# RuntimeRacer/vall-e

Hardware: AMD Instinct MI355X
Metric: AR codec-tokens/sec/GPU + NAR 7-stage p50 latency, d=1024 L=12 10s utterance (higher is better)
Workload: dtype bf16

## Files before the change

vall-e_amd/csrc/common.hpp:

```cpp
#pragma once
#include <hip/hip_runtime.h>
#include <stdint.h>

#ifdef VX_STAMPS
extern __device__ unsigned long long g_vx_stamps[32];
#define VX_STAMP(i)                                                                                        \
  do {                                                                                                     \
    if (blockIdx.x == 0 && blockIdx.y == 0 && blockIdx.z == 0 && threadIdx.x == 0) g_vx_stamps[i] = wall_clock64(); \
  } while (0)
extern __device__ unsigned long long* g_vx_kstamps;
#define VX_KSTAMP_WG(kid, st_ptr)                                                                                  \
  do {                                                                                                             \
    if ((kid) >= 0 && (kid) < 64 && blockIdx.x == gridDim.x - 1) {                                                 \
      unsigned long long* vx_r_ = g_vx_kstamps;                                                                    \
      if (vx_r_ != nullptr && threadIdx.x == 0)                                                                    \
        vx_r_[(size_t)(((st_ptr)->pass) & 15) * 64 + (kid)] = __builtin_amdgcn_s_memrealtime();                   \
      return;                                                                                                      \
    }                                                                                                              \
  } while (0)
#define VX_KSTAMP_SELF(kid, pass, t0)                                                                              \
  do {                                                                                                             \
    unsigned long long* vx_r_ = g_vx_kstamps;                                                                      \
    if (vx_r_ != nullptr && (kid) >= 0 && (kid) < 64 && threadIdx.x == 0) vx_r_[(size_t)((pass) & 15) * 64 + (kid)] = (t0); \
  } while (0)
constexpr int VX_KSTAMP_EXTRA = 1;
#else
#define VX_STAMP(i) do { } while (0)
#define VX_KSTAMP_WG(kid, st_ptr) do { } while (0)
#define VX_KSTAMP_SELF(kid, pass, t0) do { } while (0)
constexpr int VX_KSTAMP_EXTRA = 0;
#endif

namespace vx {

inline int vx_cur_device() {
  int d = 0;
  (void)hipGetDevice(&d);
  return (d < 0 || d >= 16) ? 0 : d;
}
inline int vx_cu_count() {
  static int cu[16] = {};
  const int d = vx_cur_device();
  if (cu[d] <= 0) {
    int n = 256;
    (void)hipDeviceGetAttribute(&n, hipDeviceAttributeMultiprocessorCount, d);
    cu[d] = n > 0 ? n : 256;
  }
  return cu[d];
// ... 10 lines not shown
__device__ __forceinline__ float to_f32(bf16 v) { return (float)v; }
template <typename T> __device__ __forceinline__ T from_f32(float v);
template <> __device__ __forceinline__ float from_f32<float>(float v) { return v; }
template <> __device__ __forceinline__ bf16 from_f32<bf16>(float v) { return (bf16)v; }

template <typename T> struct Vec16;
template <> struct Vec16<float> { static constexpr int N = 4; };
template <> struct Vec16<bf16> { static constexpr int N = 8; };

__device__ __forceinline__ void unpack16(const uint4& r, float (&o)[4], float*) {
  o[0] = __uint_as_float(r.x); o[1] = __uint_as_float(r.y); o[2] = __uint_as_float(r.z); o[3] = __uint_as_float(r.w);
}
__device__ __forceinline__ void unpack16(const uint4& r, float (&o)[8], bf16*) {
  o[0] = __uint_as_float(r.x << 16); o[1] = __uint_as_float(r.x & 0xffff0000u);
  o[2] = __uint_as_float(r.y << 16); o[3] = __uint_as_float(r.y & 0xffff0000u);
  o[4] = __uint_as_float(r.z << 16); o[5] = __uint_as_float(r.z & 0xffff0000u);
  o[6] = __uint_as_float(r.w << 16); o[7] = __uint_as_float(r.w & 0xffff0000u);
}
template <typename T> __device__ __forceinline__ void unpack(const uint4& r, float (&o)[Vec16<T>::N]) {
  unpack16(r, o, (T*)nullptr);
}
template <typename T> __device__ __forceinline__ uint4 ld16(const T* p) { return *reinterpret_cast<const uint4*>(p); }
typedef unsigned vx_u32x4 __attribute__((ext_vector_type(4)));

template <int CTRL, int ROW_MASK = 0xF> __device__ __forceinline__ float dpp_f(float old, float v) {
  return __builtin_bit_cast(float, __builtin_amdgcn_update_dpp(__builtin_bit_cast(int, old), __builtin_bit_cast(int, v),
                                                                CTRL, ROW_MASK, 0xF, false));
}
template <int CTRL, int ROW_MASK = 0xF> __device__ __forceinline__ int dpp_i(int old, int v) {
  return __builtin_amdgcn_update_dpp(old, v, CTRL, ROW_MASK, 0xF, false);
}
__device__ __forceinline__ float lane63(float v) {
  return __builtin_bit_cast(float, __builtin_amdgcn_readlane(__builtin_bit_cast(int, v), 63));
}
__device__ __forceinline__ float wave_sum_dpp(float v) {
  v += dpp_f<0xB1>(0.f, v);
  v += dpp_f<0x4E>(0.f, v);
  v += dpp_f<0x124>(0.f, v);
  v += dpp_f<0x128>(0.f, v);
  v += dpp_f<0x142, 0xA>(0.f, v);
  v += dpp_f<0x143, 0xC>(0.f, v);
  return lane63(v);
}
__device__ __forceinline__ float wave_max_dpp(float v) {
  v = fmaxf(v, dpp_f<0xB1>(v, v));
  v = fmaxf(v, dpp_f<0x4E>(v, v));
// ... 127 lines not shown
```

vall-e_amd/csrc/engine.hip:

```cpp
#include <hip/hip_runtime.h>

#include <cmath>
#include <cstdarg>
#include <cstdio>
#include <array>
#include <cstring>
#include <string>
#include <type_traits>
#include <unordered_map>
#include <vector>

#include "host.hpp"
#ifdef VX_STAMPS
__device__ unsigned long long g_vx_stamps[32];
__device__ unsigned long long* g_vx_kstamps = nullptr;
__device__ unsigned long long* g_fq_stamps = nullptr;
#endif
#include "ar_kernels.hpp"
#include "ar_tp.hpp"
#include "rows_kernels.hpp"
#include "mfma_kernels.hpp"
#include "batch_kernels.hpp"
#include "mx_kernels.hpp"
#include "logprob.hpp"
#include "align.hpp"

using namespace vx;

static thread_local std::string g_err;
int vx::fail(int code, const char* fmt, ...) {
  char buf[512];
  va_list ap;
  va_start(ap, fmt);
  vsnprintf(buf, sizeof buf, fmt, ap);
  va_end(ap);
  g_err = buf;
  return code;
}

// ... 3296 lines not shown
```

vall-e_amd/csrc/mfma_kernels.hpp:

```cpp
#pragma once
#include <cstdlib>
#include <type_traits>
#include <unordered_map>

#include "common.hpp"
#include "rows_kernels.hpp"

namespace vx {

typedef __bf16 bf16x8_t __attribute__((ext_vector_type(8)));
typedef float f32x16_t __attribute__((ext_vector_type(16)));

template <int EPI, bool OUT_F32, int RING>
__global__ __launch_bounds__(256) void mfma_gemm_kernel(const bf16* __restrict__ A, const bf16* __restrict__ W,
                                                        const float* __restrict__ bias, void* __restrict__ Cv, int M,
                                                        int N, int K, bf16* __restrict__ vt, int vt_n0, int vt_ld, int ld) {
  const int bx = blockIdx.x, by = blockIdx.y, bz = blockIdx.z;
  A += (size_t)bz * K;
  W += (size_t)bz * K;
  if (OUT_F32) Cv = reinterpret_cast<float*>(Cv) + (size_t)bz * M * N;
  constexpr int BM = 128, BN = 128;
  extern __shared__ __attribute__((aligned(16))) unsigned char lds[];
  const int tid = threadIdx.x, lane = tid & 63, wave = tid >> 6;
  const int wm = wave >> 1, wn = wave & 1;
  const int r = lane & 31, h = lane >> 5;
  const int m0 = by * BM, n0 = bx * BN;

  f32x16_t acc[2][2];
#pragma unroll
  for (int i = 0; i < 2; ++i)
#pragma unroll
    for (int j = 0; j < 2; ++j)
#pragma unroll
      for (int v = 0; v < 16; ++v) acc[i][j][v] = 0.f;
  float bias_r[2] = {0.f, 0.f};
  if (EPI != GE_PLAIN) {
#pragma unroll
    for (int j = 0; j < 2; ++j) bias_r[j] = bias[min(n0 + wn * 64 + j * 32 + r, N - 1)];
  }

  constexpr int RK = RING;
  constexpr int RB = RK * 2;
  constexpr int CPR = RB / 16;
  constexpr int KS = RK / 16;
  constexpr int OPB = BM * RB;
  constexpr int NI = OPB / 4096;
  constexpr int ND = 2 * NI;
  auto swz = [](int row) { return RB == 128 ? ((row >> 1) & 7) : ((0 - (row >> 2)) & 3); };
  const int nk = K / RK;
  const int row0 = tid / CPR;
  const int csrc = ((tid % CPR) ^ swz(row0)) * 8;
  const bf16 *sA[NI], *sW[NI];
#pragma unroll
  for (int i = 0; i < NI; ++i) {
    sA[i] = A + (size_t)min(m0 + row0 + (256 / CPR) * i, M - 1) * ld + csrc;
    sW[i] = W + (size_t)min(n0 + row0 + (256 / CPR) * i, N - 1) * ld + csrc;
  }
  const int dbase = (tid - lane) * 16;
  auto stage = [&](int st) {
    unsigned char* base = lds + (st & 3) * (2 * OPB);
    const int k0 = st * RK;
#pragma unroll
    for (int i = 0; i < NI; ++i)
      __builtin_amdgcn_global_load_lds((const __attribute__((address_space(1))) void*)(sA[i] + k0),
                                       (__attribute__((address_space(3))) void*)(base + dbase + 4096 * i), 16, 0, 0);
#pragma unroll
    for (int i = 0; i < NI; ++i)
      __builtin_amdgcn_global_load_lds((const __attribute__((address_space(1))) void*)(sW[i] + k0),
                                       (__attribute__((address_space(3))) void*)(base + OPB + dbase + 4096 * i), 16, 0, 0);
  };
  bf16x8_t fa0[KS][2], fb0[KS][2], fa1[KS][2], fb1[KS][2];
  auto lread = [&](int st, bf16x8_t (&fa)[KS][2], bf16x8_t (&fb)[KS][2]) {
    const unsigned char* ba = lds + (st & 3) * (2 * OPB);
    const unsigned char* bw = ba + OPB;
#pragma unroll
    for (int ks = 0; ks < KS; ++ks)
#pragma unroll
      for (int i = 0; i < 2; ++i) {
        const int row = wm * 64 + i * 32 + r;
        fa[ks][i] = *reinterpret_cast<const bf16x8_t*>(ba + row * RB + (((ks * 2 + h) ^ swz(row)) << 4));
        const int col = wn * 64 + i * 32 + r;
        fb[ks][i] = *reinterpret_cast<const bf16x8_t*>(bw + col * RB + (((ks * 2 + h) ^ swz(col)) << 4));
      }
  };
  auto mm = [&](const bf16x8_t (&fa)[KS][2], const bf16x8_t (&fb)[KS][2]) {
#pragma unroll
    for (int ks = 0; ks < KS; ++ks)
#pragma unroll
      for (int i = 0; i < 2; ++i)
#pragma unroll
        for (int j = 0; j < 2; ++j) acc[i][j] = __builtin_amdgcn_mfma_f32_32x32x16_bf16(fa[ks][i], fb[ks][j], acc[i][j], 0, 0, 0);
  };
  auto steady = [&](int st, bf16x8_t (&fa)[KS][2], bf16x8_t (&fb)[KS][2], bf16x8_t (&na)[KS][2], bf16x8_t (&nb)[KS][2]) {
    stage(st + 3);
    lread(st + 1, na, nb);
    mm(fa, fb);
#pragma unroll
    for (int i = 0; i < ND; ++i) {
      __builtin_amdgcn_sched_group_barrier(0x010, 1, 0);
      __builtin_amdgcn_sched_group_barrier(0x008, 1, 0);
    }
#pragma unroll
    for (int i = 0; i < 4 * KS - ND; ++i) {
      __builtin_amdgcn_sched_group_barrier(0x100, 4 * KS / (4 * KS - ND), 0);
      __builtin_amdgcn_sched_group_barrier(0x008, 1, 0);
    }
    if (ND == 8) asm volatile("s_waitcnt vmcnt(8)\n\ts_barrier" ::: "memory");
    else asm volatile("s_waitcnt vmcnt(4)\n\ts_barrier" ::: "memory");
  };
  auto tail = [&](int st, bf16x8_t (&fa)[KS][2], bf16x8_t (&fb)[KS][2], bf16x8_t (&na)[KS][2], bf16x8_t (&nb)[KS][2]) {
    const bool more = st + 3 < nk;
    if (more) stage(st + 3);
    if (st + 1 < nk) lread(st + 1, na, nb);
    mm(fa, fb);
    if (more && ND == 8) asm volatile("s_waitcnt vmcnt(8)\n\ts_barrier" ::: "memory");
    else if (more) asm volatile("s_waitcnt vmcnt(4)\n\ts_barrier" ::: "memory");
    else asm volatile("s_waitcnt vmcnt(0)\n\ts_barrier" ::: "memory");
  };
  VX_STAMP(0);
  const int pre = nk < 3 ? nk : 3;
  for (int st = 0; st < pre; ++st) stage(st);
  VX_STAMP(1);
  if (pre == 3 && ND == 8) asm volatile("s_waitcnt vmcnt(8)\n\ts_barrier" ::: "memory");
  else if (pre == 3) asm volatile("s_waitcnt vmcnt(4)\n\ts_barrier" ::: "memory");
  else asm volatile("s_waitcnt vmcnt(0)\n\ts_barrier" ::: "memory");
  lread(0, fa0, fb0);
  VX_STAMP(2);
  int st = 0;
  for (; st + 4 < nk; st += 2) {
    steady(st, fa0, fb0, fa1, fb1);
    steady(st + 1, fa1, fb1, fa0, fb0);
  }
  VX_STAMP(3);
  for (; st < nk; st += 2) {
    tail(st, fa0, fb0, fa1, fb1);
    if (st + 1 < nk) tail(st + 1, fa1, fb1, fa0, fb0);
  }
  VX_STAMP(4);
  asm volatile("" : "+v"(bias_r[0]), "+v"(bias_r[1]));

  if constexpr (!OUT_F32) {
    constexpr int LDT = 136;
    bf16* tile = reinterpret_cast<bf16*>(lds);
#pragma unroll
    for (int j = 0; j < 2; ++j) {
      const int nl = wn * 64 + j * 32 + r;
      const float bv = bias_r[j];
#pragma unroll
      for (int i = 0; i < 2; ++i)
#pragma unroll
        for (int v = 0; v < 16; ++v) {
          const int ml = wm * 64 + i * 32 + (v & 3) + 8 * (v >> 2) + 4 * h;
          float x = acc[i][j][v] + bv;
          if (EPI == GE_RELU) x = fmaxf(x, 0.f);
          tile[ml * LDT + nl] = (bf16)x;
        }
    }
    __syncthreads();
    bf16* C = reinterpret_cast<bf16*>(Cv);
#pragma unroll
    for (int q = 0; q < 8; ++q) {
      const int id = tid + 256 * q, row = id >> 4, c = id & 15;
      if (m0 + row < M)
        *reinterpret_cast<uint4*>(C + (size_t)(m0 + row) * N + n0 + c * 8) = *reinterpret_cast<const uint4*>(tile + row * LDT + c * 8);
    }
    if (vt != nullptr && n0 >= vt_n0) {
#pragma unroll
      for (int q = 0; q < 8; ++q) {
        const int id = tid + 256 * q, nl = id >> 4, mc = id & 15;
        union { bf16 e[8]; uint4 u; } pk;
#pragma unroll
        for (int k = 0; k < 8; ++k) pk.e[k] = tile[(mc * 8 + k) * LDT + nl];
        *reinterpret_cast<uint4*>(vt + (size_t)(n0 + nl - vt_n0) * vt_ld + m0 + mc * 8) = pk.u;
      }
    }
  } else if (m0 + BM <= M && n0 + BN <= N) {
    float* cbase = reinterpret_cast<float*>(Cv) + (size_t)(m0 + wm * 64 + 4 * h) * N + n0 + wn * 64 + r;
    float old[2][2][16];
    if (EPI == GE_RESID) {
#pragma unroll
      for (int j = 0; j < 2; ++j)
#pragma unroll
        for (int i = 0; i < 2; ++i)
#pragma unroll
          for (int v = 0; v < 16; ++v) old[i][j][v] = cbase[(size_t)(i * 32 + (v & 3) + 8 * (v >> 2)) * N + j * 32];
    }
#pragma unroll
    for (int j = 0; j < 2; ++j) {
      const float bv = bias_r[j];
#pragma unroll
      for (int i = 0; i < 2; ++i)
#pragma unroll
        for (int v = 0; v < 16; ++v) {
          float x = acc[i][j][v] + bv;
          if (EPI == GE_RELU) x = fmaxf(x, 0.f);
          if (EPI == GE_RESID) x += old[i][j][v];
          cbase[(size_t)(i * 32 + (v & 3) + 8 * (v >> 2)) * N + j * 32] = x;
        }
    }
  } else {
#pragma unroll
    for (int j = 0; j < 2; ++j) {
      const int n = n0 + wn * 64 + j * 32 + r;
      const float bv = bias_r[j];
#pragma unroll
      for (int i = 0; i < 2; ++i) {
#pragma unroll
        for (int v = 0; v < 16; ++v) {
          const int m = m0 + wm * 64 + i * 32 + (v & 3) + 8 * (v >> 2) + 4 * h;
          if (m < M && n < N) {
            float x = acc[i][j][v] + bv;
            if (EPI == GE_RELU) x = fmaxf(x, 0.f);
            float* c = reinterpret_cast<float*>(Cv) + (size_t)m * N + n;
            *c = (EPI == GE_RESID) ? (*c + x) : x;
          }
        }
      }
    }
  }
  VX_STAMP(5);
}

template <int EPI, bool OUT_F32, int SPLITK>
__global__ __launch_bounds__(256) void wgemm_kernel(const bf16* __restrict__ A, const bf16* __restrict__ W,
                                                    const float* __restrict__ bias, void* __restrict__ Cv, int M, int N,
                                                    int K, bf16* __restrict__ vt, int vt_n0, int vt_ld, int ngroups,
                                                    int ngroups_pad) {
  extern __shared__ __attribute__((aligned(16))) unsigned char lds[];
  const int tid = threadIdx.x, lane = tid & 63, wave = tid >> 6;
  const int r = lane & 31, h = lane >> 5;
  const int ng = blockIdx.x % ngroups_pad, mt = blockIdx.x / ngroups_pad;
  if (ng >= ngroups) return;
  const int m0 = mt * 64;
  const int n0 = (SPLITK == 1) ? (ng * 4 + wave) * 64 : ng * 64;
  const int kbeg = (SPLITK == 1) ? 0 : wave * (K / SPLITK);
  const int nk = (K / SPLITK) / 64;
  unsigned char* my = lds + wave * 32768;
  const bool active = n0 < N;

  f32x16_t acc[2][2];
#pragma unroll
  for (int i = 0; i < 2; ++i)
#pragma unroll
// ... 582 lines not shown
    };
    if (is_tail) {
      unsigned lo = (unsigned)((r * 256 + 4 * g) * 4);
      asm volatile("" : "+v"(lo));
      unsigned char* slab = reinterpret_cast<unsigned char*>(tl.ws + (size_t)(tail_a * S + tail_s) * 65536 + wr * 32768 + wc * 64) + lo;
#pragma unroll
      for (int i = 0; i < 8; ++i)
#pragma unroll
        for (int j = 0; j < 4; ++j) *reinterpret_cast<f32x4v_t*>(slab + i * 16384 + j * 64) = acc[i][j];
      lax = 0;
    } else if (full) {
      emit(std::false_type{});
      lax = __builtin_amdgcn_readfirstlane((has_vt || EPI == GE_RESID) ? 0 : 1);
    } else {
      emit(std::true_type{});
      lax = 0;
    }
  }
  asm volatile("s_waitcnt vmcnt(0)" ::: "memory");
  if (wr == 0) asm volatile("s_barrier" ::: "memory");
}

static inline int gemm_ring128(long long wgs) { return wgs <= vx_cu_count() ? 64 : 32; }

static inline P8Tail p8_tail_plan(int ntiles, int grid, int K, hipStream_t s) {
  static const bool on = [] { const char* v = getenv("VX_GEMM_TAIL"); return v && atoi(v) != 0; }();
  P8Tail tl{nullptr, 0};
  if (!on || ntiles <= grid || grid > 256) return tl;
  const int rem = ntiles % grid, nk = K / 64;
  if (rem == 0 || rem * 2 > grid) return tl;
  int S = 0;
  for (int c = 8; c >= 2; c >>= 1)
    if (rem * c <= grid && nk % (2 * c) == 0 && nk / c >= 8) { S = c; break; }
  if (S == 0) return tl;
  const float full = 1.5f * nk, split = 1.5f * nk / S + (float)rem * S * 0.262144f * 2.f / 4.f + 7.f;
  if (split > 0.7f * full) return tl;
  hipStreamCaptureStatus cs = hipStreamCaptureStatusNone;
  if (hipStreamIsCapturing(s, &cs) != hipSuccess || cs != hipStreamCaptureStatusNone) return tl;
  static std::unordered_map<hipStream_t, float*> wss;
  float*& w = wss[s];
  if (w == nullptr && hipMalloc((void**)&w, (size_t)256 * 262144) != hipSuccess) { w = nullptr; return tl; }
  tl.ws = w;
  tl.split = S;
  return tl;
}

// ... 16 lines not shown
      constexpr bool OUT_F32 = decltype(F)::value;
      static bool attr_dev[16] = {};
      bool& attr_done = attr_dev[vx_cur_device()];
      if (!attr_done) {
        (void)hipFuncSetAttribute((const void*)mfma256_kernel<EPI, OUT_F32>, hipFuncAttributeMaxDynamicSharedMemorySize, 131072);
        (void)hipFuncSetAttribute((const void*)mfma256p_kernel<EPI, OUT_F32>, hipFuncAttributeMaxDynamicSharedMemorySize, 131072 + 2048);
        (void)hipFuncSetAttribute((const void*)mfma256p_kernel<EPI, OUT_F32, true>, hipFuncAttributeMaxDynamicSharedMemorySize, 131072 + 2048);
        attr_done = true;
      }
      if (p8 && tl.split > 1) {
        const int rem_t = nt_all % grid256;
        mfma256p_kernel<EPI, OUT_F32, true><<<grid256, 512, 131072 + 2048, s>>>(A, W, bias, C, M, N, K, vt, vt_n0, vt_ld, ntn, nt_all, tl);
        p8_tail_reduce_kernel<EPI, OUT_F32><<<dim3(rem_t, 16), 256, 0, s>>>(tl.ws, tl.split, nt_all - rem_t, ntn, nt_all, bias, C, M, N, vt, vt_n0, vt_ld);
      } else if (p8) {
        mfma256p_kernel<EPI, OUT_F32><<<grid256, 512, 131072 + 2048, s>>>(A, W, bias, C, M, N, K, vt, vt_n0, vt_ld, ntn, nt_all, tl);
      } else {
        mfma256_kernel<EPI, OUT_F32><<<grid256, 512, 131072, s>>>(A, W, bias, C, M, N, K, vt, vt_n0, vt_ld, ntn, nt_all);
      }
    });
    return 0;
  }
  if (N % 128 == 0 && tiles64 >= 512) {
    const dim3 grid(N / 128, (M + 127) / 128);
    const int ring = gemm_ring128((long long)grid.x * grid.y);
    gemm_epi_dispatch(epi, out_f32, [&](auto E, auto F) {
      constexpr int EPI = decltype(E)::value;
      constexpr bool OUT_F32 = decltype(F)::value;
      static bool attr_dev[16] = {};
      bool& attr_done = attr_dev[vx_cur_device()];
      if (!attr_done) {
        (void)hipFuncSetAttribute((const void*)mfma_gemm_kernel<EPI, OUT_F32, 64>, hipFuncAttributeMaxDynamicSharedMemorySize, 131072);
        (void)hipFuncSetAttribute((const void*)mfma_gemm_kernel<EPI, OUT_F32, 32>, hipFuncAttributeMaxDynamicSharedMemorySize, 65536);
        attr_done = true;
      }
      if (ring == 64) mfma_gemm_kernel<EPI, OUT_F32, 64><<<grid, 256, 131072, s>>>(A, W, bias, C, M, N, K, vt, vt_n0, vt_ld, K);
      else mfma_gemm_kernel<EPI, OUT_F32, 32><<<grid, 256, 65536, s>>>(A, W, bias, C, M, N, K, vt, vt_n0, vt_ld, K);
    });
    return 0;
  }
  const int mtiles = (M + 63) / 64;
  const size_t lds = 131072;
  const bool split = (K % 256 == 0) && tiles64 < 512;
  gemm_epi_dispatch(epi, out_f32, [&](auto E, auto F) {
    constexpr int EPI = decltype(E)::value;
    constexpr bool OUT_F32 = decltype(F)::value;
    auto launch = [&](auto SPLITK) {
      constexpr int S = decltype(SPLITK)::value;
      static bool attr_dev[16] = {};
      bool& attr_done = attr_dev[vx_cur_device()];
      if (!attr_done) {
        (void)hipFuncSetAttribute((const void*)wgemm_kernel<EPI, OUT_F32, S>, hipFuncAttributeMaxDynamicSharedMemorySize, (int)lds);
        attr_done = true;
      }
      const int ngr = (S == 1) ? (N + 255) / 256 : N / 64;
      const int ngp = (ngr + 7) / 8 * 8;
      wgemm_kernel<EPI, OUT_F32, S><<<mtiles * ngp, 256, lds, s>>>(A, W, bias, C, M, N, K, vt, vt_n0, vt_ld, ngr, ngp);
    };
    if (split) launch(std::integral_constant<int, 4>{});
    else launch(std::integral_constant<int, 1>{});
  });
  return 0;
}

static inline int mfma_gemm_partial(const bf16* A, const bf16* W, float* slabs, int M, int N, int K, int splits, hipStream_t s) {
  static bool attr_dev[16] = {}; bool& attr_done = attr_dev[vx_cur_device()];
  if (!attr_done) {
    (void)hipFuncSetAttribute((const void*)mfma_gemm_kernel<GE_PLAIN, true, 64>, hipFuncAttributeMaxDynamicSharedMemorySize, 131072);
    (void)hipFuncSetAttribute((const void*)mfma_gemm_kernel<GE_PLAIN, true, 32>, hipFuncAttributeMaxDynamicSharedMemorySize, 65536);
    attr_done = true;
  }
  dim3 grid(N / 128, (M + 127) / 128, splits);
  if (gemm_ring128((long long)grid.x * grid.y * grid.z) == 64)
    mfma_gemm_kernel<GE_PLAIN, true, 64><<<grid, 256, 131072, s>>>(A, W, nullptr, slabs, M, N, K / splits, nullptr, 0, 0, K);
  else
    mfma_gemm_kernel<GE_PLAIN, true, 32><<<grid, 256, 65536, s>>>(A, W, nullptr, slabs, M, N, K / splits, nullptr, 0, 0, K);
  return 0;
}

__device__ __forceinline__ float xor32_f(float v) {
  const auto r = __builtin_amdgcn_permlane32_swap(__builtin_bit_cast(unsigned, v), __builtin_bit_cast(unsigned, v), false, false);
  return __builtin_bit_cast(float, (threadIdx.x & 32) ? r[0] : r[1]);
}

template <int NW, int KG>
__global__ __launch_bounds__(NW * KG * 64, (KG == 2 ? 2 : 1)) void mfma_attn_kernel(const bf16* __restrict__ qkv, const bf16* __restrict__ vt,
                                                                 bf16* __restrict__ out, int M, int vt_ld, int d,
                                                                 int text_len, const int* __restrict__ seg_start,
                                                                 const int* __restrict__ seg_len,
                                                                 const int* __restrict__ seg_text) {
  constexpr int HD = 64, NT = NW * KG * 64;
  int bx, by, bz;
  {
    const unsigned gx = gridDim.x, gy = gridDim.y, total = gx * gy * gridDim.z;
    const unsigned lin = blockIdx.x + gx * (blockIdx.y + gy * blockIdx.z);
    const unsigned n8 = total >> 3;
    const unsigned logical = lin < (n8 << 3) ? (lin & 7u) * n8 + (lin >> 3) : lin;
    bx = (int)(logical % gx);
    by = (int)((logical / gx) % gy);
// ... 225 lines not shown
#pragma unroll
      for (int t = 0; t < 2; ++t)
#pragma unroll
        for (int v = 0; v < 16; v += 4) *reinterpret_cast<float4*>(p + 4 + t * 16 + v) = make_float4(accO[t][v], accO[t][v + 1], accO[t][v + 2], accO[t][v + 3]);
    }
    __syncthreads();
    if (kg > 0) return;
#pragma unroll
    for (int g = 1; g < KG; ++g) {
      const float* p = park + ((size_t)((g - 1) * NW + qw) * 64 + lane) * 36;
      const float m1 = p[0], l1 = p[1];
      const float mm = fmaxf(m_run, m1);
      const float f0 = (m_run == -INFINITY) ? 0.f : __expf(m_run - mm), f1 = (m1 == -INFINITY) ? 0.f : __expf(m1 - mm);
      l_tot = l_tot * f0 + l1 * f1;
#pragma unroll
      for (int t = 0; t < 2; ++t)
#pragma unroll
        for (int v = 0; v < 16; ++v) accO[t][v] = accO[t][v] * f0 + p[4 + t * 16 + v] * f1;
      m_run = mm;
    }
  }
  if (qvalid) {
    const float inv = 1.0f / l_tot;
    bf16* op = out + (size_t)qrow * d + head * HD;
#pragma unroll
    for (int t = 0; t < 2; ++t)
#pragma unroll
      for (int g4 = 0; g4 < 4; ++g4) {
        union { bf16 b[4]; uint2 u; } pk;
#pragma unroll
        for (int j = 0; j < 4; ++j) pk.b[j] = (bf16)(accO[t][4 * g4 + j] * inv);
        *reinterpret_cast<uint2*>(op + t * 32 + 8 * g4 + 4 * hh) = pk.u;
      }
  }
  VX_STAMP(23);
}

__global__ __launch_bounds__(256) void vt_from_qkv_kernel(const bf16* __restrict__ qkv, bf16* __restrict__ vt, int M, int d,
                                                          int vt_ld) {
  const int m = blockIdx.x * 256 + threadIdx.x, c = blockIdx.y;
  if (m < vt_ld) vt[(size_t)c * vt_ld + m] = (m < M) ? qkv[(size_t)m * 3 * d + 2 * d + c] : (bf16)0.f;
}

static inline int mfma_attn_dispatch(const bf16* qkv, const bf16* vt, int vt_ld, bf16* out, int M, int d, int H,
                                     int text_len, hipStream_t s, const int* seg_start = nullptr,
                                     const int* seg_len = nullptr, int nseg = 1, int max_seg_len = 0,
                                     const int* seg_text = nullptr) {
  const int rows = seg_start ? max_seg_len : M;
  if ((unsigned long long)rows * 3ull * d * 2ull >= (1ull << 32) || (unsigned long long)d * vt_ld * 2ull >= (1ull << 32)) return 1;
  static bool attr_dev[16] = {}; bool& attr_done = attr_dev[vx_cur_device()];
  if (!attr_done) {
    (void)hipFuncSetAttribute((const void*)mfma_attn_kernel<2, 2>, hipFuncAttributeMaxDynamicSharedMemorySize, 65536);
    attr_done = true;
  }
  const long long nwg2 = (long long)((rows + 63) / 64) * H * (seg_start ? nseg : 1);
// ... 187 lines not shown
```

vall-e_amd/csrc/probe_entry.hpp:

```cpp
#pragma once
#include "persist_probe.hpp"
#include "probes.h"

__global__ void noop_kernel(float* p) {
  if (p != nullptr && threadIdx.x == 0 && blockIdx.x == 0x7fffffff) p[0] = 0.f;
}

extern "C" int vx_debug_launch_floor(int32_t n_kernels, int32_t grid, int32_t block, int32_t iters, double* out) {
  if (!out || n_kernels <= 0 || iters <= 0) return fail(VX_ERR_ARG, "bad argument");
  hipStream_t s;
  HIPC(hipStreamCreateWithFlags(&s, hipStreamNonBlocking));
  hipEvent_t e0, e1;
  HIPC(hipEventCreate(&e0));
  HIPC(hipEventCreate(&e1));
  hipGraph_t g;
  hipGraphExec_t ge;
  HIPC(hipStreamBeginCapture(s, hipStreamCaptureModeThreadLocal));
  for (int i = 0; i < n_kernels; ++i) noop_kernel<<<grid, block, 0, s>>>(nullptr);
  HIPC(hipStreamEndCapture(s, &g));
  HIPC(hipGraphInstantiate(&ge, g, nullptr, nullptr, 0));
  for (int i = 0; i < 3; ++i) HIPC(hipGraphLaunch(ge, s));
  HIPC(hipStreamSynchronize(s));
  float ms = 0.f;
  HIPC(hipEventRecord(e0, s));
// ... 188 lines not shown
#endif
}

extern "C" int vx_debug_fqstamps(void* dst, int64_t nbytes) {
#ifdef VX_STAMPS
  static unsigned long long* buf = nullptr;
  const size_t bytes = (size_t)2 * 16 * 256 * 16 * 8;
  HIPC(hipDeviceSynchronize());
  if (dst == nullptr) {
    if (!buf) HIPC(hipMalloc((void**)&buf, bytes));
    HIPC(hipMemset(buf, 0, bytes));
    HIPC(hipMemcpyToSymbol(HIP_SYMBOL(g_fq_stamps), &buf, sizeof buf));
    HIPC(hipDeviceSynchronize());
    return VX_OK;
  }
  if (!buf) return fail(VX_ERR_STATE, "stamps not armed");
  HIPC(hipMemcpy(dst, buf, (size_t)nbytes < bytes ? (size_t)nbytes : bytes, hipMemcpyDeviceToHost));
  return VX_OK;
#else
  (void)dst; (void)nbytes;
  return fail(VX_ERR_UNSUPPORTED, "library built without -DVX_STAMPS");
#endif
}
```

vall-e_amd/csrc/probes.h:

```cpp
#ifndef VALLEX_PROBES_H
#define VALLEX_PROBES_H
#include <stdint.h>
#ifdef __cplusplus
extern "C" {
#endif

int vx_debug_launch_floor(int32_t n_kernels, int32_t grid, int32_t block, int32_t iters, double* out);
int vx_debug_stage_chain(int32_t nwg, int32_t stages, int32_t rows, int32_t mode, int32_t iters, double* out);
int vx_debug_l2_fill(int32_t grid, int32_t threads, int32_t unroll, int64_t region_bytes, int32_t iters, double* out);
int vx_debug_read_stamps(unsigned long long* out, int32_t n);
int vx_debug_kstamps(void* dst, int64_t nbytes, int32_t* dims);

int vx_debug_fqstamps(void* dst, int64_t nbytes);

#ifdef __cplusplus
}
#endif
#endif
```

vall-e_amd/csrc/rows_kernels.hpp:

```cpp
#pragma once
#include <type_traits>

#include "common.hpp"

namespace vx {

__global__ __launch_bounds__(256) void embed_pos_kernel(const long long* __restrict__ ids, int id_stride, int id_off,
                                                        const float* __restrict__ table, int table_rows, int d,
                                                        const float* __restrict__ alpha, const float* __restrict__ pe,
                                                        int pos0, float* __restrict__ out, int rows) {
  const int r = blockIdx.x;
  if (r >= rows) return;
  const long long id = min(max(ids[(size_t)r * id_stride + id_off], 0ll), (long long)table_rows - 1);
  const float al = alpha[0];
  for (int c = threadIdx.x; c < d; c += 256)
    out[(size_t)r * d + c] = __fadd_rn(table[(size_t)id * d + c], __fmul_rn(al, pe[(size_t)(pos0 + r) * d + c]));
}

__global__ __launch_bounds__(256) void add_pos_kernel(const float* __restrict__ src, int d,
                                                      const float* __restrict__ alpha, const float* __restrict__ pe,
                                                      int pos0, float* __restrict__ out, int rows) {
  const int r = blockIdx.x;
  if (r >= rows) return;
  const float al = alpha[0];
// ... 45 lines not shown
      if (t0 + j >= S) break;
      const float v = (acc[j] + bias[co] - bn_mean[co]) * inv * bn_g[co] + bn_b[co];
      y[(size_t)(t0 + j) * d + co] = fmaxf(v, 0.f);
    }
  }
}

__global__ __launch_bounds__(256) void conv_weight_relayout_kernel(const float* __restrict__ w, float* __restrict__ wt, int d) {
  const size_t n = (size_t)d * d * 5, i = (size_t)blockIdx.x * 256 + threadIdx.x;
  if (i >= n) return;
  const int k = (int)(i % 5), ci = (int)((i / 5) % d), co = (int)(i / (5 * (size_t)d));
  wt[((size_t)k * d + ci) * d + co] = w[i];
}

template <typename OT, int MAXV>
__global__ __launch_bounds__(256) void layernorm_rows_kernel(const float* x, const float* __restrict__ gamma,
                                                             const float* __restrict__ beta,
                                                             const float* __restrict__ ada_w,
                                                             const float* __restrict__ ada_b, OT* __restrict__ out,
                                                             int rows, int d, float* xout = nullptr,
                                                             const float* __restrict__ part = nullptr, int nsplit = 0,
                                                             size_t part_stride = 0, const float* __restrict__ pbias = nullptr) {
  const int lane = threadIdx.x & 63;
  const int r = blockIdx.x * 4 + (threadIdx.x >> 6);
  if (r >= rows) return;
  const float* xr = x + (size_t)r * d;
  const bool fold = part != nullptr, norm = out != nullptr, ada = ada_w != nullptr;
  float4 v[MAXV], g[MAXV], b[MAXV], w[MAXV], c[MAXV];
  int kk[MAXV];
  bool ok[MAXV];
#pragma unroll
  for (int i = 0; i < MAXV; ++i) {
    const int k = (i * 64 + lane) * 4;
    ok[i] = k < d;
    kk[i] = ok[i] ? k : 0;
    v[i] = *reinterpret_cast<const float4*>(xr + kk[i]);
    if (norm) {
      g[i] = *reinterpret_cast<const float4*>(gamma + kk[i]);
      b[i] = *reinterpret_cast<const float4*>(beta + kk[i]);
      if (ada) {
        w[i] = *reinterpret_cast<const float4*>(ada_w + kk[i]);
        c[i] = *reinterpret_cast<const float4*>(ada_b + kk[i]);
      }
    }
  }
  if (fold) {
#pragma unroll
    for (int i = 0; i < MAXV; ++i) {
      float4 t = *reinterpret_cast<const float4*>(pbias + kk[i]);
      float4 p[4];
#pragma unroll
      for (int z = 0; z < 4; ++z)
        p[z] = *reinterpret_cast<const float4*>(part + (size_t)min(z, nsplit - 1) * part_stride + (size_t)r * d + kk[i]);
#pragma unroll
      for (int z = 0; z < 4; ++z)
        if (z < nsplit) { t.x += p[z].x; t.y += p[z].y; t.z += p[z].z; t.w += p[z].w; }
      v[i].x += t.x; v[i].y += t.y; v[i].z += t.z; v[i].w += t.w;
      if (ok[i] && (xout == nullptr || !norm)) *reinterpret_cast<float4*>(const_cast<float*>(xr) + kk[i]) = v[i];
    }
  }
  if (!norm) return;
  float s = 0.f;
#pragma unroll
  for (int i = 0; i < MAXV; ++i) s += ok[i] ? (v[i].x + v[i].y) + (v[i].z + v[i].w) : 0.f;
  const float mean = wave_sum(s) / (float)d;
  float ss = 0.f;
#pragma unroll
  for (int i = 0; i < MAXV; ++i) {
    const float d0 = v[i].x - mean, d1 = v[i].y - mean, d2 = v[i].z - mean, d3 = v[i].w - mean;
    ss += ok[i] ? (d0 * d0 + d1 * d1) + (d2 * d2 + d3 * d3) : 0.f;
  }
  const float rstd = 1.0f / sqrtf(wave_sum(ss) / (float)d + LN_EPS);
#pragma unroll
  for (int i = 0; i < MAXV; ++i) {
    if (!ok[i]) continue;
    float o[4] = {(v[i].x - mean) * rstd * g[i].x + b[i].x, (v[i].y - mean) * rstd * g[i].y + b[i].y,
                  (v[i].z - mean) * rstd * g[i].z + b[i].z, (v[i].w - mean) * rstd * g[i].w + b[i].w};
    if (ada) {
      o[0] = __fadd_rn(__fmul_rn(w[i].x, o[0]), c[i].x); o[1] = __fadd_rn(__fmul_rn(w[i].y, o[1]), c[i].y);
      o[2] = __fadd_rn(__fmul_rn(w[i].z, o[2]), c[i].z); o[3] = __fadd_rn(__fmul_rn(w[i].w, o[3]), c[i].w);
    }
    union { OT e[4]; uint2 u2; float4 f4; } pk;
#pragma unroll
    for (int j = 0; j < 4; ++j) pk.e[j] = from_f32<OT>(o[j]);
    OT* op = out + (size_t)r * d + kk[i];
    if (sizeof(OT) == 2) *reinterpret_cast<uint2*>(op) = pk.u2;
    else *reinterpret_cast<float4*>(op) = pk.f4;
    if (xout != nullptr) *reinterpret_cast<float4*>(xout + (size_t)r * d + kk[i]) = make_float4(o[0], o[1], o[2], o[3]);
  }
}

__global__ __launch_bounds__(256) void project_vec_kernel(const float* __restrict__ W, const float* __restrict__ b,
                                                          const float* __restrict__ e, float* __restrict__ out,
                                                          int N, int K) {
  const int lane = threadIdx.x & 63;
  const int row = blockIdx.x * 4 + (threadIdx.x >> 6);
  if (row >= N) return;
  float s = 0.f;
  for (int k = lane; k < K; k += 64) s = fmaf(W[(size_t)row * K + k], e[k], s);
  s = wave_sum(s);
  if (lane == 0) out[row] = s + b[row];
}

enum GemmEpi { GE_PLAIN = 0, GE_BIAS = 1, GE_RELU = 2, GE_RESID = 3 };

template <class F>
static inline void gemm_epi_dispatch(int epi, bool out_f32, F&& f) {
  using std::integral_constant;
  if (epi == GE_RESID) f(integral_constant<int, GE_RESID>{}, std::true_type{});
  else if (epi == GE_PLAIN) f(integral_constant<int, GE_PLAIN>{}, std::true_type{});
  else if (epi == GE_BIAS && out_f32) f(integral_constant<int, GE_BIAS>{}, std::true_type{});
// ... 358 lines not shown
```

Measured before the change: 4583.

## Add configurable GEMM LDS ring slots and write-through buffer stores for outputs

Generalizes the MFMA GEMM LDS ring from a fixed four stages to a compile-time SLOTS count, with counted vmcnt waits expressed by template helpers. It also adds buffer-resource store helpers that pass a cache-policy bit, applied selectively via VX_WT_MASK. By default only the fp32 GEMM outputs use it, so split-K slabs and residual results bypass or stream through cache for the consumers that follow. It also adds stage-level timing probes under VX_STAMPS, and uses readfirstlane for the row index in the layernorm kernel. The write-through stores risk different cache behavior for data reread soon after.

```diff
diff --git a/vall-e_amd/csrc/common.hpp b/vall-e_amd/csrc/common.hpp
--- a/vall-e_amd/csrc/common.hpp
+++ b/vall-e_amd/csrc/common.hpp
@@ -24,6 +24,8 @@
     if (vx_r_ != nullptr && (kid) >= 0 && (kid) < 64 && threadIdx.x == 0) vx_r_[(size_t)((pass) & 15) * 64 + (kid)] = (t0); \
   } while (0)
 constexpr int VX_KSTAMP_EXTRA = 1;
+extern __device__ unsigned long long* g_vx_stage_stamps;
+constexpr int VX_STAGE_STAMP_WGS = 1024;
 #else
 #define VX_STAMP(i) do { } while (0)
 #define VX_KSTAMP_WG(kid, st_ptr) do { } while (0)
@@ -80,6 +82,25 @@
 }
 template <typename T> __device__ __forceinline__ uint4 ld16(const T* p) { return *reinterpret_cast<const uint4*>(p); }
 typedef unsigned vx_u32x4 __attribute__((ext_vector_type(4)));
+
+typedef __amdgpu_buffer_rsrc_t vx_window;
+__device__ __forceinline__ vx_window wt_window(void* base) { return __builtin_amdgcn_make_buffer_rsrc(base, 0, 0x7fffffff, 0x00020000); }
+template <bool WT> __device__ __forceinline__ void st16_wt(vx_window w, void* base, unsigned off, const uint4& v) {
+  if (WT) __builtin_amdgcn_raw_buffer_store_b128(vx_u32x4{v.x, v.y, v.z, v.w}, w, (int)off, 0, 16);
+  else *reinterpret_cast<uint4*>(reinterpret_cast<unsigned char*>(base) + off) = v;
+}
+template <bool WT> __device__ __forceinline__ void st8_wt(vx_window w, void* base, unsigned off, const uint2& v) {
+  typedef unsigned u32x2 __attribute__((ext_vector_type(2)));
+  if (WT) __builtin_amdgcn_raw_buffer_store_b64(u32x2{v.x, v.y}, w, (int)off, 0, 16);
+  else *reinterpret_cast<uint2*>(reinterpret_cast<unsigned char*>(base) + off) = v;
+}
+template <bool WT> __device__ __forceinline__ void st4_wt(vx_window w, void* base, unsigned off, float v) {
+  if (WT) __builtin_amdgcn_raw_buffer_store_b32(__float_as_uint(v), w, (int)off, 0, 16);
+  else *reinterpret_cast<float*>(reinterpret_cast<unsigned char*>(base) + off) = v;
+}
+#ifndef VX_WT_MASK
+#define VX_WT_MASK 2
+#endif
 
 template <int CTRL, int ROW_MASK = 0xF> __device__ __forceinline__ float dpp_f(float old, float v) {
   return __builtin_bit_cast(float, __builtin_amdgcn_update_dpp(__builtin_bit_cast(int, old), __builtin_bit_cast(int, v),
diff --git a/vall-e_amd/csrc/engine.hip b/vall-e_amd/csrc/engine.hip
--- a/vall-e_amd/csrc/engine.hip
+++ b/vall-e_amd/csrc/engine.hip
@@ -15,6 +15,7 @@
 __device__ unsigned long long g_vx_stamps[32];
 __device__ unsigned long long* g_vx_kstamps = nullptr;
 __device__ unsigned long long* g_fq_stamps = nullptr;
+__device__ unsigned long long* g_vx_stage_stamps = nullptr;
 #endif
 #include "ar_kernels.hpp"
 #include "ar_tp.hpp"
diff --git a/vall-e_amd/csrc/mfma_kernels.hpp b/vall-e_amd/csrc/mfma_kernels.hpp
--- a/vall-e_amd/csrc/mfma_kernels.hpp
+++ b/vall-e_amd/csrc/mfma_kernels.hpp
@@ -11,7 +11,16 @@
 typedef __bf16 bf16x8_t __attribute__((ext_vector_type(8)));
 typedef float f32x16_t __attribute__((ext_vector_type(16)));
 
-template <int EPI, bool OUT_F32, int RING>
+template <int CNT> __device__ __forceinline__ void ring_wait_barrier() {
+  asm volatile("s_waitcnt vmcnt(%0)\n\ts_barrier" ::"n"(CNT) : "memory");
+}
+template <int ND, int JMAX> __device__ __forceinline__ void ring_wait_younger(int j) {
+  if constexpr (JMAX <= 0) ring_wait_barrier<0>();
+  else if (j >= JMAX) ring_wait_barrier<ND * JMAX>();
+  else ring_wait_younger<ND, JMAX - 1>(j);
+}
+
+template <int EPI, bool OUT_F32, int RING, int SLOTS>
 __global__ __launch_bounds__(256) void mfma_gemm_kernel(const bf16* __restrict__ A, const bf16* __restrict__ W,
                                                         const float* __restrict__ bias, void* __restrict__ Cv, int M,
                                                         int N, int K, bf16* __restrict__ vt, int vt_n0, int vt_ld, int ld) {
@@ -21,10 +30,17 @@
   if (OUT_F32) Cv = reinterpret_cast<float*>(Cv) + (size_t)bz * M * N;
   constexpr int BM = 128, BN = 128;
   extern __shared__ __attribute__((aligned(16))) unsigned char lds[];
+  static_assert(SLOTS >= 4 && SLOTS * RING * 512 <= 163840, "at least 4 slots, at most 160 KB of LDS");
+  static_assert(RING / 8 * (SLOTS - 3) < 64, "the counted wait must fit the 6-bit vmcnt");
   const int tid = threadIdx.x, lane = tid & 63, wave = tid >> 6;
   const int wm = wave >> 1, wn = wave & 1;
   const int r = lane & 31, h = lane >> 5;
   const int m0 = by * BM, n0 = bx * BN;
+#ifdef VX_STAMPS
+  unsigned long long sst[8] = {};
+  sst[4] = __builtin_amdgcn_s_memtime();
+  sst[6] = __builtin_amdgcn_s_memrealtime();
+#endif
 
   f32x16_t acc[2][2];
 #pragma unroll
@@ -57,8 +73,11 @@
     sW[i] = W + (size_t)min(n0 + row0 + (256 / CPR) * i, N - 1) * ld + csrc;
   }
   const int dbase = (tid - lane) * 16;
+  auto nxt = [](int slot) { return slot + 1 == SLOTS ? 0 : slot + 1; };
+  int si = 0, sr = 0;
   auto stage = [&](int st) {
-    unsigned char* base = lds + (st & 3) * (2 * OPB);
+    unsigned char* base = lds + si * (2 * OPB);
+    si = nxt(si);
     const int k0 = st * RK;
 #pragma unroll
     for (int i = 0; i < NI; ++i)
@@ -70,9 +89,10 @@
                                        (__attribute__((address_space(3))) void*)(base + OPB + dbase + 4096 * i), 16, 0, 0);
   };
   bf16x8_t fa0[KS][2], fb0[KS][2], fa1[KS][2], fb1[KS][2];
-  auto lread = [&](int st, bf16x8_t (&fa)[KS][2], bf16x8_t (&fb)[KS][2]) {
-    const unsigned char* ba = lds + (st & 3) * (2 * OPB);
+  auto lread = [&](bf16x8_t (&fa)[KS][2], bf16x8_t (&fb)[KS][2]) {
+    const unsigned char* ba = lds + sr * (2 * OPB);
     const unsigned char* bw = ba + OPB;
+    sr = nxt(sr);
 #pragma unroll
     for (int ks = 0; ks < KS; ++ks)
 #pragma unroll
@@ -91,9 +111,16 @@
 #pragma unroll
         for (int j = 0; j < 2; ++j) acc[i][j] = __builtin_amdgcn_mfma_f32_32x32x16_bf16(fa[ks][i], fb[ks][j], acc[i][j], 0, 0, 0);
   };
-  auto steady = [&](int st, bf16x8_t (&fa)[KS][2], bf16x8_t (&fb)[KS][2], bf16x8_t (&na)[KS][2], bf16x8_t (&nb)[KS][2]) {
-    stage(st + 3);
-    lread(st + 1, na, nb);
+  constexpr int AHEAD = SLOTS - 1;
+  auto steady = [&](auto STAMPED, int st, bf16x8_t (&fa)[KS][2], bf16x8_t (&fb)[KS][2], bf16x8_t (&na)[KS][2], bf16x8_t (&nb)[KS][2]) {
+#ifdef VX_STAMPS
+    if (decltype(STAMPED)::value) {
+      sst[0] = __builtin_amdgcn_s_memtime();
+      __builtin_amdgcn_sched_barrier(0);
+    }
+#endif
+    stage(st + AHEAD);
+    lread(na, nb);
     mm(fa, fb);
 #pragma unroll
     for (int i = 0; i < ND; ++i) {
@@ -105,31 +132,46 @@
       __builtin_amdgcn_sched_group_barrier(0x100, 4 * KS / (4 * KS - ND), 0);
       __builtin_amdgcn_sched_group_barrier(0x008, 1, 0);
     }
-    if (ND == 8) asm volatile("s_waitcnt vmcnt(8)\n\ts_barrier" ::: "memory");
-    else asm volatile("s_waitcnt vmcnt(4)\n\ts_barrier" ::: "memory");
+#ifdef VX_STAMPS
+    if (decltype(STAMPED)::value) {
+      __builtin_amdgcn_sched_barrier(0);
+      sst[1] = __builtin_amdgcn_s_memtime();
+      __builtin_amdgcn_sched_barrier(0);
+      asm volatile("s_waitcnt vmcnt(%0)" ::"n"(ND * (SLOTS - 3)) : "memory");
+      sst[2] = __builtin_amdgcn_s_memtime();
+      __builtin_amdgcn_sched_barrier(0);
+      asm volatile("s_barrier" ::: "memory");
+      sst[3] = __builtin_amdgcn_s_memtime();
+      __builtin_amdgcn_sched_barrier(0);
+      return;
+    }
+#endif
+    ring_wait_barrier<ND * (SLOTS - 3)>();
   };
   auto tail = [&](int st, bf16x8_t (&fa)[KS][2], bf16x8_t (&fb)[KS][2], bf16x8_t (&na)[KS][2], bf16x8_t (&nb)[KS][2]) {
-    const bool more = st + 3 < nk;
-    if (more) stage(st + 3);
-    if (st + 1 < nk) lread(st + 1, na, nb);
+    if (st + AHEAD < nk) stage(st + AHEAD);
+    if (st + 1 < nk) lread(na, nb);
     mm(fa, fb);
-    if (more && ND == 8) asm volatile("s_waitcnt vmcnt(8)\n\ts_barrier" ::: "memory");
-    else if (more) asm volatile("s_waitcnt vmcnt(4)\n\ts_barrier" ::: "memory");
-    else asm volatile("s_waitcnt vmcnt(0)\n\ts_barrier" ::: "memory");
+    ring_wait_younger<ND, SLOTS - 3>(min(st + AHEAD, nk - 1) - (st + 2));
   };
   VX_STAMP(0);
-  const int pre = nk < 3 ? nk : 3;
+  const int pre = nk < AHEAD ? nk : AHEAD;
   for (int st = 0; st < pre; ++st) stage(st);
   VX_STAMP(1);
-  if (pre == 3 && ND == 8) asm volatile("s_waitcnt vmcnt(8)\n\ts_barrier" ::: "memory");
-  else if (pre == 3) asm volatile("s_waitcnt vmcnt(4)\n\ts_barrier" ::: "memory");
-  else asm volatile("s_waitcnt vmcnt(0)\n\ts_barrier" ::: "memory");
-  lread(0, fa0, fb0);
+  ring_wait_younger<ND, SLOTS - 3>(pre - 2);
+  lread(fa0, fb0);
   VX_STAMP(2);
   int st = 0;
-  for (; st + 4 < nk; st += 2) {
-    steady(st, fa0, fb0, fa1, fb1);
-    steady(st + 1, fa1, fb1, fa0, fb0);
+#ifdef VX_STAMPS
+  const int st_stamp = ((nk - SLOTS) / 2) & ~1;
+#endif
+  for (; st + SLOTS < nk; st += 2) {
+#ifdef VX_STAMPS
+    if (st == st_stamp) steady(std::true_type{}, st, fa0, fb0, fa1, fb1);
+    else
+#endif
+    steady(std::false_type{}, st, fa0, fb0, fa1, fb1);
+    steady(std::false_type{}, st + 1, fa1, fb1, fa0, fb0);
   }
   VX_STAMP(3);
   for (; st < nk; st += 2) {
@@ -157,25 +199,32 @@
         }
     }
     __syncthreads();
-    bf16* C = reinterpret_cast<bf16*>(Cv);
+    constexpr bool WT = (VX_WT_MASK & 1) != 0;
+    bf16* cb = reinterpret_cast<bf16*>(Cv) + (size_t)m0 * N + n0;
+    const vx_window cw = wt_window(cb);
 #pragma unroll
     for (int q = 0; q < 8; ++q) {
       const int id = tid + 256 * q, row = id >> 4, c = id & 15;
-      if (m0 + row < M)
-        *reinterpret_cast<uint4*>(C + (size_t)(m0 + row) * N + n0 + c * 8) = *reinterpret_cast<const uint4*>(tile + row * LDT + c * 8);
+      if (m0 + row < M) st16_wt<WT>(cw, cb, (unsigned)(row * N + c * 8) * 2u, *reinterpret_cast<const uint4*>(tile + row * LDT + c * 8));
     }
     if (vt != nullptr && n0 >= vt_n0) {
+      bf16* vb = vt + (size_t)(n0 - vt_n0) * vt_ld + m0;
+      const vx_window vw = wt_window(vb);
 #pragma unroll
       for (int q = 0; q < 8; ++q) {
         const int id = tid + 256 * q, nl = id >> 4, mc = id & 15;
         union { bf16 e[8]; uint4 u; } pk;
 #pragma unroll
         for (int k = 0; k < 8; ++k) pk.e[k] = tile[(mc * 8 + k) * LDT + nl];
-        *reinterpret_cast<uint4*>(vt + (size_t)(n0 + nl - vt_n0) * vt_ld + m0 + mc * 8) = pk.u;
+        st16_wt<WT>(vw, vb, (unsigned)(nl * vt_ld + mc * 8) * 2u, pk.u);
       }
     }
   } else if (m0 + BM <= M && n0 + BN <= N) {
-    float* cbase = reinterpret_cast<float*>(Cv) + (size_t)(m0 + wm * 64 + 4 * h) * N + n0 + wn * 64 + r;
+    constexpr bool WT = (VX_WT_MASK & 2) != 0;
+    float* tb = reinterpret_cast<float*>(Cv) + (size_t)m0 * N + n0;
+    const vx_window tw = wt_window(tb);
+    const int coff = (wm * 64 + 4 * h) * N + wn * 64 + r;
+    float* cbase = tb + coff;
     float old[2][2][16];
     if (EPI == GE_RESID) {
 #pragma unroll
@@ -195,30 +244,45 @@
           float x = acc[i][j][v] + bv;
           if (EPI == GE_RELU) x = fmaxf(x, 0.f);
           if (EPI == GE_RESID) x += old[i][j][v];
-          cbase[(size_t)(i * 32 + (v & 3) + 8 * (v >> 2)) * N + j * 32] = x;
+          st4_wt<WT>(tw, tb, (unsigned)(coff + (i * 32 + (v & 3) + 8 * (v >> 2)) * N + j * 32) * 4u, x);
         }
     }
   } else {
+    constexpr bool WT = (VX_WT_MASK & 2) != 0;
+    float* tb = reinterpret_cast<float*>(Cv) + (size_t)m0 * N + n0;
+    const vx_window tw = wt_window(tb);
 #pragma unroll
     for (int j = 0; j < 2; ++j) {
-      const int n = n0 + wn * 64 + j * 32 + r;
+      const int nl = wn * 64 + j * 32 + r;
       const float bv = bias_r[j];
 #pragma unroll
       for (int i = 0; i < 2; ++i) {
 #pragma unroll
         for (int v = 0; v < 16; ++v) {
-          const int m = m0 + wm * 64 + i * 32 + (v & 3) + 8 * (v >> 2) + 4 * h;
-          if (m < M && n < N) {
+          const int ml = wm * 64 + i * 32 + (v & 3) + 8 * (v >> 2) + 4 * h;
+          if (m0 + ml < M && n0 + nl < N) {
             float x = acc[i][j][v] + bv;
             if (EPI == GE_RELU) x = fmaxf(x, 0.f);
-            float* c = reinterpret_cast<float*>(Cv) + (size_t)m * N + n;
-            *c = (EPI == GE_RESID) ? (*c + x) : x;
+            const float* c = tb + (size_t)ml * N + nl;
+            st4_wt<WT>(tw, tb, (unsigned)(ml * N + nl) * 4u, (EPI == GE_RESID) ? (*c + x) : x);
           }
         }
       }
     }
   }
   VX_STAMP(5);
+#ifdef VX_STAMPS
+  {
+    sst[5] = __builtin_amdgcn_s_memtime();
+    sst[7] = __builtin_amdgcn_s_memrealtime();
+    unsigned long long* dst = g_vx_stage_stamps;
+    const int wg = bx + gridDim.x * (by + gridDim.y * bz);
+    if (dst != nullptr && wg < VX_STAGE_STAMP_WGS && lane == 0) {
+#pragma unroll
+      for (int i = 0; i < 8; ++i) dst[((size_t)wg * 4 + wave) * 8 + i] = sst[i];
+    }
+  }
+#endif
 }
 
 template <int EPI, bool OUT_F32, int SPLITK>
@@ -847,6 +911,35 @@
 }
 
 static inline int gemm_ring128(long long wgs) { return wgs <= vx_cu_count() ? 64 : 32; }
+#ifndef VX_RING1_K
+#define VX_RING1_K 64
+#endif
+#ifndef VX_RING1_SLOTS
+#define VX_RING1_SLOTS 4
+#endif
+#ifndef VX_RING2_SLOTS
+#define VX_RING2_SLOTS 4
+#endif
+constexpr int RING1_K = VX_RING1_K, RING1_SLOTS = VX_RING1_SLOTS;
+constexpr int RING2_K = 32, RING2_SLOTS = VX_RING2_SLOTS;
+static_assert(RING2_K * RING2_SLOTS * 512 <= 81920, "two workgroups of the two-per-CU form must fit a CU's 160 KB of LDS");
+
+template <int EPI, bool OUT_F32>
+static inline void mfma_gemm128_launch(dim3 grid, hipStream_t s, const bf16* A, const bf16* W, const float* bias, void* C, int M, int N,
+                                       int K, bf16* vt, int vt_n0, int vt_ld, int ld) {
+  constexpr int LDS1 = RING1_K * RING1_SLOTS * 512, LDS2 = RING2_K * RING2_SLOTS * 512;
+  static bool attr_dev[16] = {};
+  bool& attr_done = attr_dev[vx_cur_device()];
+  if (!attr_done) {
+    (void)hipFuncSetAttribute((const void*)mfma_gemm_kernel<EPI, OUT_F32, RING1_K, RING1_SLOTS>, hipFuncAttributeMaxDynamicSharedMemorySize, LDS1);
+    (void)hipFuncSetAttribute((const void*)mfma_gemm_kernel<EPI, OUT_F32, RING2_K, RING2_SLOTS>, hipFuncAttributeMaxDynamicSharedMemorySize, LDS2);
+    attr_done = true;
+  }
+  if (gemm_ring128((long long)grid.x * grid.y * grid.z) == 64)
+    mfma_gemm_kernel<EPI, OUT_F32, RING1_K, RING1_SLOTS><<<grid, 256, LDS1, s>>>(A, W, bias, C, M, N, K, vt, vt_n0, vt_ld, ld);
+  else
+    mfma_gemm_kernel<EPI, OUT_F32, RING2_K, RING2_SLOTS><<<grid, 256, LDS2, s>>>(A, W, bias, C, M, N, K, vt, vt_n0, vt_ld, ld);
+}
 
 static inline P8Tail p8_tail_plan(int ntiles, int grid, int K, hipStream_t s) {
   static const bool on = [] { const char* v = getenv("VX_GEMM_TAIL"); return v && atoi(v) != 0; }();
@@ -909,19 +1002,8 @@
   }
   if (N % 128 == 0 && tiles64 >= 512) {
     const dim3 grid(N / 128, (M + 127) / 128);
-    const int ring = gemm_ring128((long long)grid.x * grid.y);
     gemm_epi_dispatch(epi, out_f32, [&](auto E, auto F) {
-      constexpr int EPI = decltype(E)::value;
-      constexpr bool OUT_F32 = decltype(F)::value;
-      static bool attr_dev[16] = {};
-      bool& attr_done = attr_dev[vx_cur_device()];
-      if (!attr_done) {
-        (void)hipFuncSetAttribute((const void*)mfma_gemm_kernel<EPI, OUT_F32, 64>, hipFuncAttributeMaxDynamicSharedMemorySize, 131072);
-        (void)hipFuncSetAttribute((const void*)mfma_gemm_kernel<EPI, OUT_F32, 32>, hipFuncAttributeMaxDynamicSharedMemorySize, 65536);
-        attr_done = true;
-      }
-      if (ring == 64) mfma_gemm_kernel<EPI, OUT_F32, 64><<<grid, 256, 131072, s>>>(A, W, bias, C, M, N, K, vt, vt_n0, vt_ld, K);
-      else mfma_gemm_kernel<EPI, OUT_F32, 32><<<grid, 256, 65536, s>>>(A, W, bias, C, M, N, K, vt, vt_n0, vt_ld, K);
+      mfma_gemm128_launch<decltype(E)::value, decltype(F)::value>(grid, s, A, W, bias, C, M, N, K, vt, vt_n0, vt_ld, K);
     });
     return 0;
   }
@@ -950,17 +1032,7 @@
 }
 
 static inline int mfma_gemm_partial(const bf16* A, const bf16* W, float* slabs, int M, int N, int K, int splits, hipStream_t s) {
-  static bool attr_dev[16] = {}; bool& attr_done = attr_dev[vx_cur_device()];
-  if (!attr_done) {
-    (void)hipFuncSetAttribute((const void*)mfma_gemm_kernel<GE_PLAIN, true, 64>, hipFuncAttributeMaxDynamicSharedMemorySize, 131072);
-    (void)hipFuncSetAttribute((const void*)mfma_gemm_kernel<GE_PLAIN, true, 32>, hipFuncAttributeMaxDynamicSharedMemorySize, 65536);
-    attr_done = true;
-  }
-  dim3 grid(N / 128, (M + 127) / 128, splits);
-  if (gemm_ring128((long long)grid.x * grid.y * grid.z) == 64)
-    mfma_gemm_kernel<GE_PLAIN, true, 64><<<grid, 256, 131072, s>>>(A, W, nullptr, slabs, M, N, K / splits, nullptr, 0, 0, K);
-  else
-    mfma_gemm_kernel<GE_PLAIN, true, 32><<<grid, 256, 65536, s>>>(A, W, nullptr, slabs, M, N, K / splits, nullptr, 0, 0, K);
+  mfma_gemm128_launch<GE_PLAIN, true>(dim3(N / 128, (M + 127) / 128, splits), s, A, W, nullptr, slabs, M, N, K / splits, nullptr, 0, 0, K);
   return 0;
 }
 
@@ -1232,7 +1304,9 @@
   }
   if (qvalid) {
     const float inv = 1.0f / l_tot;
-    bf16* op = out + (size_t)qrow * d + head * HD;
+    constexpr bool WT = (VX_WT_MASK & 8) != 0;
+    const vx_window ow = wt_window(out);
+    const unsigned op = (unsigned)(qrow * d + head * HD);
 #pragma unroll
     for (int t = 0; t < 2; ++t)
 #pragma unroll
@@ -1240,7 +1314,7 @@
         union { bf16 b[4]; uint2 u; } pk;
 #pragma unroll
         for (int j = 0; j < 4; ++j) pk.b[j] = (bf16)(accO[t][4 * g4 + j] * inv);
-        *reinterpret_cast<uint2*>(op + t * 32 + 8 * g4 + 4 * hh) = pk.u;
+        st8_wt<WT>(ow, out, (op + t * 32 + 8 * g4 + 4 * hh) * 2u, pk.u);
       }
   }
   VX_STAMP(23);
diff --git a/vall-e_amd/csrc/probe_entry.hpp b/vall-e_amd/csrc/probe_entry.hpp
--- a/vall-e_amd/csrc/probe_entry.hpp
+++ b/vall-e_amd/csrc/probe_entry.hpp
@@ -234,3 +234,24 @@
   return fail(VX_ERR_UNSUPPORTED, "library built without -DVX_STAMPS");
 #endif
 }
+
+extern "C" int vx_debug_gemm_stage_stamps(void* dst, int64_t nbytes) {
+#ifdef VX_STAMPS
+  static unsigned long long* buf = nullptr;
+  const size_t bytes = (size_t)VX_STAGE_STAMP_WGS * 4 * 8 * 8;
+  HIPC(hipDeviceSynchronize());
+  if (dst == nullptr) {
+    if (!buf) HIPC(hipMalloc((void**)&buf, bytes));
+    HIPC(hipMemset(buf, 0, bytes));
+    HIPC(hipMemcpyToSymbol(HIP_SYMBOL(g_vx_stage_stamps), &buf, sizeof buf));
+    HIPC(hipDeviceSynchronize());
+    return VX_OK;
+  }
+  if (!buf) return fail(VX_ERR_STATE, "stamps not armed");
+  HIPC(hipMemcpy(dst, buf, (size_t)nbytes < bytes ? (size_t)nbytes : bytes, hipMemcpyDeviceToHost));
+  return VX_OK;
+#else
+  (void)dst; (void)nbytes;
+  return fail(VX_ERR_UNSUPPORTED, "library built without -DVX_STAMPS");
+#endif
+}
diff --git a/vall-e_amd/csrc/probes.h b/vall-e_amd/csrc/probes.h
--- a/vall-e_amd/csrc/probes.h
+++ b/vall-e_amd/csrc/probes.h
@@ -12,6 +12,7 @@
 int vx_debug_kstamps(void* dst, int64_t nbytes, int32_t* dims);
 
 int vx_debug_fqstamps(void* dst, int64_t nbytes);
+int vx_debug_gemm_stage_stamps(void* dst, int64_t nbytes);
 
 #ifdef __cplusplus
 }
diff --git a/vall-e_amd/csrc/rows_kernels.hpp b/vall-e_amd/csrc/rows_kernels.hpp
--- a/vall-e_amd/csrc/rows_kernels.hpp
+++ b/vall-e_amd/csrc/rows_kernels.hpp
@@ -91,10 +91,15 @@
                                                              const float* __restrict__ part = nullptr, int nsplit = 0,
                                                              size_t part_stride = 0, const float* __restrict__ pbias = nullptr) {
   const int lane = threadIdx.x & 63;
-  const int r = blockIdx.x * 4 + (threadIdx.x >> 6);
+  const int r = __builtin_amdgcn_readfirstlane(blockIdx.x * 4 + (threadIdx.x >> 6));
   if (r >= rows) return;
   const float* xr = x + (size_t)r * d;
   const bool fold = part != nullptr, norm = out != nullptr, ada = ada_w != nullptr;
+  constexpr bool WT = (VX_WT_MASK & 4) != 0;
+  float* xw = const_cast<float*>(xr);
+  OT* ow = out + (size_t)r * d;
+  float* xow = xout + (size_t)r * d;
+  const vx_window wx = wt_window(xw), wo = wt_window(ow), wxo = wt_window(xow);
   float4 v[MAXV], g[MAXV], b[MAXV], w[MAXV], c[MAXV];
   int kk[MAXV];
   bool ok[MAXV];
@@ -125,7 +130,7 @@
       for (int z = 0; z < 4; ++z)
         if (z < nsplit) { t.x += p[z].x; t.y += p[z].y; t.z += p[z].z; t.w += p[z].w; }
       v[i].x += t.x; v[i].y += t.y; v[i].z += t.z; v[i].w += t.w;
-      if (ok[i] && (xout == nullptr || !norm)) *reinterpret_cast<float4*>(const_cast<float*>(xr) + kk[i]) = v[i];
+      if (ok[i] && (xout == nullptr || !norm)) st16_wt<WT>(wx, xw, kk[i] * 4u, make_uint4(__float_as_uint(v[i].x), __float_as_uint(v[i].y), __float_as_uint(v[i].z), __float_as_uint(v[i].w)));
     }
   }
   if (!norm) return;
@@ -149,13 +154,12 @@
       o[0] = __fadd_rn(__fmul_rn(w[i].x, o[0]), c[i].x); o[1] = __fadd_rn(__fmul_rn(w[i].y, o[1]), c[i].y);
       o[2] = __fadd_rn(__fmul_rn(w[i].z, o[2]), c[i].z); o[3] = __fadd_rn(__fmul_rn(w[i].w, o[3]), c[i].w);
     }
-    union { OT e[4]; uint2 u2; float4 f4; } pk;
+    union { OT e[4]; uint2 u2; uint4 u4; } pk;
 #pragma unroll
     for (int j = 0; j < 4; ++j) pk.e[j] = from_f32<OT>(o[j]);
-    OT* op = out + (size_t)r * d + kk[i];
-    if (sizeof(OT) == 2) *reinterpret_cast<uint2*>(op) = pk.u2;
-    else *reinterpret_cast<float4*>(op) = pk.f4;
-    if (xout != nullptr) *reinterpret_cast<float4*>(xout + (size_t)r * d + kk[i]) = make_float4(o[0], o[1], o[2], o[3]);
+    if (sizeof(OT) == 2) st8_wt<WT>(wo, ow, kk[i] * 2u, pk.u2);
+    else st16_wt<WT>(wo, ow, kk[i] * 4u, pk.u4);
+    if (xout != nullptr) st16_wt<WT>(wxo, xow, kk[i] * 4u, make_uint4(__float_as_uint(o[0]), __float_as_uint(o[1]), __float_as_uint(o[2]), __float_as_uint(o[3])));
   }
 }
 
```

Result: no change. 4583, median of 3 (+0.0%).
